# reglab/aquaculture

Measured on AMD Instinct MI355X. Metric: 640px tiles/sec (whole node) YOLOv5m bf16, higher is better.
Workload: dtype bf16

## Files before the change

### aquaculture_amd/csrc/conv1x1_direct.hip

```cpp
#include "conv_device.h"

using namespace aqdev;

namespace {

struct C1Params {
    const char* in;
    char* out;
    const char* w;
    const float* bias;
    const char* zero;
    int in_ld_b, out_ld_b;
    int npix, n_tiles, act;
    float out_inv_scale;
};

constexpr int kNW = 12;

template <int KS, int MBT, int MBW, int NBW> struct C1Geom {
    static constexpr int CIN = 32 * KS, COUT = 16 * MBT, CB = CIN / 8;
    static constexpr int MG = MBT / MBW;
    static constexpr int PG = kNW / MG;
    static constexpr int TP = PG * NBW * 16;
    static constexpr int SPP = CB + 2;
    static constexpr int PXB = SPP * 16;
    static constexpr int NQ = (TP * SPP + 63) / 64;
    static constexpr int XPB = NQ * 1024;
    static constexpr int LDS = 2 * XPB + COUT * 4;
    static constexpr int NST = NBW;
    static_assert(MBT % MBW == 0 && kNW % MG == 0 && LDS <= 160 * 1024, "shape");
};

__device__ __forceinline__ f32x4 c1_silu4(f32x4 v) {
    const f32x4 t = v * -1.44269504f;
    f32x4 d = {__builtin_amdgcn_exp2f(t[0]), __builtin_amdgcn_exp2f(t[1]), __builtin_amdgcn_exp2f(t[2]), __builtin_amdgcn_exp2f(t[3])};
    d = d + 1.0f;
    const f32x4 r = {__builtin_amdgcn_rcpf(d[0]), __builtin_amdgcn_rcpf(d[1]), __builtin_amdgcn_rcpf(d[2]), __builtin_amdgcn_rcpf(d[3])};
    return v * r;
}

template <int KS, int MBT, int MBW, int NBW, bool F8OUT = false>
__global__ __launch_bounds__(kNW * 64) void conv1x1_direct_kernel(const C1Params p) {
    using G = C1Geom<KS, MBT, MBW, NBW>;
    extern __shared__ __attribute__((aligned(16))) char smem[];
    float* s_b = (float*)(smem + 2 * G::XPB);

    const int tid = threadIdx.x, lane = tid & 63;
    const int wave = __builtin_amdgcn_readfirstlane(tid >> 6);
    static_assert(MBW == 2, "the paired-row layout below is written for two M blocks per wave");
    const int mb0 = (wave % G::MG) * MBW, pg = wave / G::MG;
    const int g = lane >> 4, l15 = lane & 15;
    const int cbase = mb0 * 16 + g * 8;

    bf16x8 wv[KS][MBW];
#pragma unroll
    for (int s = 0; s < KS; ++s)
#pragma unroll
        for (int m = 0; m < MBW; ++m) wv[s][m] = ((const bf16x8*)p.w)[((size_t)(mb0 + m) * KS + s) * 64 + lane];
    for (int i = tid; i < G::COUT; i += kNW * 64) s_b[i] = p.bias[i];

    auto issue_dma = [&](int tile, char* xb) {
        const long long n0 = (long long)tile * G::TP;
#pragma unroll 1
        for (int q = wave; q < G::NQ; q += kNW) {
            const int slot = q * 64 + lane;
            const int px = slot / G::SPP, part = slot - px * G::SPP;
            const bool valid = px < G::TP && part < G::CB && n0 + px < p.npix;
            const char* src = p.in + (n0 + px) * p.in_ld_b + part * 16;
            glds16(valid ? src : p.zero, xb + q * 1024);
        }
    };

    int tile = first_tile(gridDim.x, blockIdx.x);
    if (tile < p.n_tiles) issue_dma(tile, smem);
    int cur = 0;
    bool prev_full = false;
    for (; tile < p.n_tiles; tile += gridDim.x, cur ^= 1) {
        const long long n0 = (long long)tile * G::TP;
        const char* s_x = smem + cur * G::XPB;
        if (prev_full) wait_vmcnt<G::NST>(); else wait_vmcnt<0>();
        asm volatile("s_waitcnt lgkmcnt(0)" ::: "memory");
        __builtin_amdgcn_s_barrier();
        asm volatile("" ::: "memory");
        prev_full = n0 + G::TP <= p.npix;
        if (tile + (int)gridDim.x < p.n_tiles) issue_dma(tile + (int)gridDim.x, smem + (cur ^ 1) * G::XPB);

        f32x4 bv[MBW];
#pragma unroll
        for (int m = 0; m < MBW; ++m) bv[m] = *(const f32x4*)(s_b + cbase + m * 4);
        static_assert(G::NST == NBW * 1, "one 16-byte (8-byte with F8OUT) store per pixel block: the wait at the top of the tile loop counts these");
        AQ_STORE_LOOP_UNROLL
// ... 11 lines not shown
#pragma unroll
                for (int m = 0; m < MBW; ++m) acc[m] = __builtin_amdgcn_mfma_f32_16x16x32_bf16(wv[s][m], f[s], acc[m], 0, 0, 0);
            f32x4 v0 = acc[0] + bv[0], v1 = acc[1] + bv[1];
            if (p.act) { v0 = c1_silu4(v0); v1 = c1_silu4(v1); }
            if constexpr (F8OUT) {
                f32x4 q0 = v0 * p.out_inv_scale, q1 = v1 * p.out_inv_scale;
#pragma unroll
                for (int e = 0; e < 4; ++e) {
                    q0[e] = __builtin_amdgcn_fmed3f(q0[e], -448.0f, 448.0f);
                    q1[e] = __builtin_amdgcn_fmed3f(q1[e], -448.0f, 448.0f);
                }
                int w0 = __builtin_amdgcn_cvt_pk_fp8_f32(q0[0], q0[1], 0, false);
                w0 = __builtin_amdgcn_cvt_pk_fp8_f32(q0[2], q0[3], w0, true);
                int w1 = __builtin_amdgcn_cvt_pk_fp8_f32(q1[0], q1[1], 0, false);
                w1 = __builtin_amdgcn_cvt_pk_fp8_f32(q1[2], q1[3], w1, true);
                if (n0 + px < p.npix) *(uint2*)(p.out + (n0 + px) * p.out_ld_b + cbase) = make_uint2((unsigned)w0, (unsigned)w1);
            } else if (n0 + px < p.npix)
                *(uint4*)(p.out + (n0 + px) * p.out_ld_b + cbase * 2) =
                    make_uint4(pack_bf16x2(v0[0], v0[1]), pack_bf16x2(v0[2], v0[3]), pack_bf16x2(v1[0], v1[1]), pack_bf16x2(v1[2], v1[3]));
        }
    }
}

template <int KS, int MBT, int MBW, int NBW, bool F8OUT = false>
int launch_c1(C1Params p, hipStream_t stream) {
    using G = C1Geom<KS, MBT, MBW, NBW>;
    auto fn = conv1x1_direct_kernel<KS, MBT, MBW, NBW, F8OUT>;
    int cus = 0;
    AQ_CHECK_HIP(aq_kernel_lds((const void*)fn, G::LDS));
    AQ_CHECK_HIP(aq_cus(&cus));
    p.n_tiles = (p.npix + G::TP - 1) / G::TP;
    long long grid = cus;
    if (grid > p.n_tiles) grid = p.n_tiles;
    hipLaunchKernelGGL(fn, dim3((unsigned)grid), dim3(kNW * 64), G::LDS, stream, p);
    AQ_CHECK_HIP(hipGetLastError());
    return AQ_OK;
}

}

extern "C" int aq_conv1x1_direct_supported(int cin, int cout) {
    return (cin == 96 && cout == 96) || (cin == 192 && cout == 192) || (cin == 384 && (cout == 192 || cout == 384));
}

extern "C" int aq_pack_conv1x1_direct(const float* w_host, int cin, int cout, void* packed_dev, size_t* bytes, void* stream) {
    AQ_REQUIRE(w_host && bytes && aq_conv1x1_direct_supported(cin, cout), "pack_conv1x1_direct: unsupported %d -> %d", cin, cout);
    const int ks = cin / 32, mbt = cout / 16;
    *bytes = (size_t)mbt * ks * 64 * 16;
    if (!packed_dev) return AQ_OK;
    bf16_t* host = (bf16_t*)calloc(1, *bytes);
    AQ_REQUIRE(host, "pack_conv1x1_direct: out of host memory");
    for (int mb = 0; mb < mbt; ++mb)
        for (int s = 0; s < ks; ++s)
            for (int lane = 0; lane < 64; ++lane) {
                const int r = lane & 15, g = lane >> 4;
                const int co = (mb >> 1) * 32 + 8 * (r >> 2) + 4 * (mb & 1) + (r & 3);
                bf16_t* dst = host + (((size_t)mb * ks + s) * 64 + lane) * 8;
                for (int e = 0; e < 8; ++e) dst[e] = aq_f2bf(w_host[(size_t)co * cin + 32 * s + 8 * g + e]);
            }
    hipError_t e = hipMemcpyAsync(packed_dev, host, *bytes, hipMemcpyHostToDevice, (hipStream_t)stream);
    if (e == hipSuccess) e = hipStreamSynchronize((hipStream_t)stream);
    free(host);
    AQ_CHECK_HIP(e);
    return AQ_OK;
}

extern "C" int aq_conv1x1_direct(const void* in_dev, int in_ld, int in_choff, void* out_dev, int out_ld, int out_choff, int cin, int cout,
                                 const void* packed_w_dev, const float* bias_dev, long long npix, int act, void* stream) {
    AQ_REQUIRE(in_dev && out_dev && packed_w_dev && bias_dev, "conv1x1_direct: null pointer");
    AQ_REQUIRE(aq_conv1x1_direct_supported(cin, cout), "conv1x1_direct: unsupported %d -> %d", cin, cout);
    AQ_REQUIRE(npix > 0 && sg::conv1x1_direct_fits(npix), "conv1x1_direct: bad pixel count");
    AQ_REQUIRE(in_ld % 8 == 0 && out_ld % 8 == 0 && in_choff % 8 == 0 && out_choff % 8 == 0 && in_choff + cin <= in_ld && out_choff + cout <= out_ld,
               "conv1x1_direct: channel slices must be 8-aligned and inside their rows");
    C1Params p{};
    p.in = (const char*)in_dev + (size_t)in_choff * 2; p.in_ld_b = in_ld * 2;
    p.out = (char*)out_dev + (size_t)out_choff * 2; p.out_ld_b = out_ld * 2;
    p.w = (const char*)packed_w_dev; p.bias = bias_dev;
    p.npix = (int)npix; p.act = act;
    p.zero = aq_zero_page();
    AQ_REQUIRE(p.zero, "conv1x1_direct: zero page allocation failed");
    const hipStream_t st = (hipStream_t)stream;
    if (cin == 96) return launch_c1<3, 6, 2, 4>(p, st);
    if (cin == 192) return launch_c1<6, 12, 2, 4>(p, st);
    if (cout == 192) return launch_c1<12, 12, 2, 2>(p, st);
    return launch_c1<12, 24, 2, 4>(p, st);
}


extern "C" int aq_conv1x1_direct_f8out(const void* in_dev, int in_ld, int in_choff, void* out_dev, int out_pitch_bytes, int out_byte_off, int cin,
                                       int cout, const void* packed_w_dev, const float* bias_dev, long long npix, int act, float out_scale,
                                       void* stream) {
    AQ_REQUIRE(in_dev && out_dev && packed_w_dev && bias_dev, "conv1x1_direct_f8out: null pointer");
    AQ_REQUIRE((cin == 192 && cout == 192) || (cin == 384 && cout == 384), "conv1x1_direct_f8out: unsupported %d -> %d", cin, cout);
    AQ_REQUIRE(npix > 0 && sg::conv1x1_direct_fits(npix) && out_scale > 0.0f, "conv1x1_direct_f8out: bad pixel count or scale");
    AQ_REQUIRE(in_ld % 8 == 0 && in_choff % 8 == 0 && in_choff + cin <= in_ld && out_pitch_bytes % 8 == 0 && out_byte_off % 8 == 0 &&
                   out_byte_off + cout <= out_pitch_bytes, "conv1x1_direct_f8out: slices must be 8-byte aligned and inside their rows");
    C1Params p{};
    p.in = (const char*)in_dev + (size_t)in_choff * 2; p.in_ld_b = in_ld * 2;
    p.out = (char*)out_dev + out_byte_off; p.out_ld_b = out_pitch_bytes;
    p.w = (const char*)packed_w_dev; p.bias = bias_dev;
    p.npix = (int)npix; p.act = act; p.out_inv_scale = 1.0f / out_scale;
    p.zero = aq_zero_page();
    AQ_REQUIRE(p.zero, "conv1x1_direct_f8out: zero page allocation failed");
    const hipStream_t st = (hipStream_t)stream;
    if (cin == 192) return launch_c1<6, 12, 2, 4, true>(p, st);
    return launch_c1<12, 24, 2, 4, true>(p, st);
}
```

### aquaculture_amd/csrc/engine.cpp

```cpp
#include "aq_common.h"
#include <unistd.h>
#include <string>

#include <cstdarg>
#include <cstdio>
#include <cstdlib>
#include <cstring>
#include <string>
#include <atomic>
#include <dlfcn.h>
#include <vector>

namespace {
thread_local char g_err[512] = "";
}

void aq_set_error(const char* fmt, ...) {
    va_list ap;
    va_start(ap, fmt);
    vsnprintf(g_err, sizeof(g_err), fmt, ap);
    va_end(ap);
}

extern "C" const char* aq_last_error(void) { return g_err; }
// ... 115 lines not shown
            }
        }
    }
    *kgroups = kg; *kgroups_pad = kgp; *G = g; *cout_rows = rows;
}

struct TensorPlace { size_t offset = 0; size_t bytes = 0; int h = 0, w = 0, elem = 0; };

}

struct aq_engine {
    int device = 0;
    aq_model_desc desc{};
    std::vector<aq_tensor_desc> tensors;
    std::vector<aq_op_desc> ops;
    std::vector<PackedW> packed;
    std::vector<int> conv_cfg;
    int nms_agnostic = 0;
    unsigned long long nms_cls_lo = ~0ULL, nms_cls_hi = ~0ULL;
    struct Tuned { int B = 0, H = 0, W = 0; std::vector<int> cfg; };
    std::vector<Tuned> tuned;
    int tuned_cur = -1;
    bool tuning = false;
    void* zero_page = nullptr;
    int lay_B = 0, lay_H = 0, lay_W = 0;
    bool lay_aug = false;
    int run_H = 0, run_W = 0;
    std::vector<TensorPlace> place;
    size_t off_pred = 0, off_cand = 0, off_cand_rows = 0, off_cand_count = 0, off_cand_wide = 0, off_nms = 0, off_taps = 0, total_bytes = 0;
    int N = 0;
    aq_augment_pass aug[3] = {};
    std::vector<int> aug_family[3], aug_cfg[3];
    void* last_ws = nullptr;
    const uint8_t* last_tiles = nullptr;
    float* calib_amax = nullptr;
    std::vector<int> last_family, last_cfg;
    bool prof = false;
    int ring = 0;
    long long prof_calls = 0;
    std::vector<hipEvent_t> ev;
};

namespace {

void set_dims(aq_engine* e, int H, int W) {
    for (size_t t = 0; t < e->tensors.size(); ++t) {
// ... 289 lines not shown
            if (!(form || igemm)) return fail(oi, "conv: %lld output pixels are past the implicit-GEMM guard (pixels < 2^24, K groups < 2^15, tile count < 2^31) and no other form takes it", npix);
            break;
        }
        default:
            break;
        }
    }
    return -1;
}

bool c3tail_active(aq_engine* e, int oi, int last, int B) {
    if (!e->packed[oi].w_tail || oi + 1 >= last || e->calib_amax || e->tuning) return false;
    const int ci = oi + 1;
    const PackedW& pc = e->packed[ci];
    if (pc.direct_cfg != AQ_CONV_CFG_DIRECT1X1 || (pc.f8_consumer >= 0 && f8_pair_active(e, pc.f8_consumer, B))) return false;
    const aq_engine::Tuned* tt = tuned_for(e);
    const int cfg = e->conv_cfg[ci] >= 0 ? e->conv_cfg[ci] : tt ? tt->cfg[ci] : -1;
    if (cfg != AQ_CONV_CFG_DIRECT1X1) return false;
    const aq_op_desc& b = e->ops[oi];
    const aq_op_desc& c = e->ops[ci];
    const TensorPlace& pl = e->place[b.src.tensor];
    return aq_bottleneck_c3tail_supported(B, pl.h, pl.w, e->tensors[b.src.tensor].channels, e->tensors[c.src.tensor].channels,
                                          e->tensors[c.dst.tensor].channels) != 0;
}

struct AugRun {
    int pass;
    const aq_augment_pass* ps;
    int H0, W0;
    const aq_tap* ytab;
    const aq_tap* xtab;
};

int run_plan(aq_engine* e, const uint8_t* tiles, int B, int H, int W, void* ws, size_t ws_bytes,
             float* pred_out, aq_det* dets, int32_t* counts, float conf, float iou, int max_det, hipStream_t stream,
             int first = 0, int last = -1, const AugRun* ar = nullptr) {
    AQ_REQUIRE(e && tiles && ws, "infer: null pointer");
    const int n_ops = (int)e->ops.size();
    if (last < 0) last = n_ops;
    AQ_REQUIRE(0 <= first && first <= last && last <= n_ops, "run_ops: range [%d, %d) is not inside the plan's %d ops", first, last, n_ops);
    int rc = AQ_OK;
    if (!ar) {
        rc = layout(e, B, H, W);
        if (rc) return rc;
        if (ws_bytes < e->total_bytes) {
            aq_set_error("workspace too small: need %zu bytes, got %zu", e->total_bytes, ws_bytes);
// ... 5 lines not shown
    const float aug_scale = ar ? ar->ps->scale : 1.0f, aug_flip_w = ar && ar->ps->flip ? (float)ar->W0 : 0.0f;
    e->last_ws = ws; e->last_tiles = tiles;
    const int prec = e->desc.precision;
    const bool whole = first == 0 && last == n_ops;
    hipEvent_t* ev = nullptr;
    if (whole && !ar && e->prof && e->ring > 0) ev = e->ev.data() + (size_t)(e->prof_calls % e->ring) * (n_ops + 1);
    float* pred = pred_out ? pred_out : (float*)((char*)ws + e->off_pred);
    int32_t* cand = (int32_t*)((char*)ws + e->off_cand);
    int32_t* cand_count = (int32_t*)((char*)ws + e->off_cand_count);
    float* cand_rows = (float*)((char*)ws + e->off_cand_rows);
    const char* use_sd = getenv("AQ_STEMDOWN");
    const bool stemdown = use_sd && *use_sd == '1' && prec == AQ_BF16 && n_ops > 2 && e->ops[0].kind == AQ_OP_STEM && e->ops[1].kind == AQ_OP_DOWNBLOCK &&
                          e->ops[0].dst.channels == 48 && e->ops[1].src.tensor == e->ops[0].dst.tensor && e->ops[1].src.ch_off == e->ops[0].dst.ch_off &&
                          aq_stemdown_supported(H, W) && ((uintptr_t)tiles & 3) == 0 && !scaled;
    const bool fuse_heads = dets != nullptr && heads_fused(e);
    bool heads_started = ar != nullptr;
    int heads_done = 0;
    for (int oi = 0; oi < first; ++oi)
        if (fuse_heads && e->ops[oi].kind == AQ_OP_CONV && e->ops[oi].level >= 0) {
            heads_started = true;
            ++heads_done;
        }
    int tail_conv = -1;
    for (int oi = first; oi < last; ++oi) {
        const aq_op_desc& op = e->ops[oi];
        if (ev) AQ_CHECK_HIP(hipEventRecord(ev[oi], stream));
        const bool mark = g_roctx.on();
        if (mark) {
            char name[96];
            snprintf(name, sizeof name, "aq op %02d kind %d: %d -> %d ch, k%d s%d%s", oi, op.kind, op.src.channels, op.dst.channels, op.k, op.stride,
                     op.level >= 0 ? " (detect head)" : "");
            g_roctx.push(name);
        }
        switch (op.kind) {
        case AQ_OP_PREPROCESS:
            if (scaled)
                rc = aq_preprocess_s2d_scaled(tiles, ar->H0, ar->W0, ar->ytab, ar->xtab, ar->ps->h, ar->ps->w, tptr(e, ws, tiles, op.dst.tensor), B, H, W,
                                              prec, stream);
            else
                rc = aq_preprocess_s2d(tiles, tptr(e, ws, tiles, op.dst.tensor), B, H, W, prec, stream);
            break;
        case AQ_OP_CONV:
            if (oi == tail_conv) {
                note_launch(e, oi, AQ_FAM_DIRECT1X1, AQ_CONV_CFG_DIRECT1X1);
                break;
            }
            if (ar && op.level >= 0 && !((ar->ps->level_mask >> op.level) & 1)) {
                note_launch(e, oi, AQ_FAM_NONE);
                break;
            }
            if (fuse_heads && op.level >= 0) {
                int32_t* wide = (int32_t*)((char*)ws + e->off_cand_wide);
                if (!heads_started) {
                    AQ_CHECK_HIP(hipMemsetAsync(wide, 0, sizeof(int32_t) * B * kCountStride, stream));
                    heads_started = true;
                }
                const TensorPlace& pl = e->place[op.src.tensor];
                int off = 0;
                for (int l = 0; l < op.level; ++l) off += e->desc.na * (H / (int)e->desc.stride[l]) * (W / (int)e->desc.stride[l]);
                float anchors[8 * 2];
                for (int a = 0; a < e->desc.na; ++a) {
                    anchors[2 * a] = e->desc.anchors_px[op.level][a][0];
                    anchors[2 * a + 1] = e->desc.anchors_px[op.level][a][1];
                }
                note_launch(e, oi, AQ_FAM_HEAD_DECODE);
                if (ar) {
                    rc = aq_head_decode_aug(tptr(e, ws, tiles, op.src.tensor), e->tensors[op.src.tensor].channels, op.src.ch_off, op.src.channels,
// ... 45 lines not shown
                               op.src.channels, e->packed[oi].w, e->packed[oi].bias, B, pl.h, pl.w, op.res.tensor >= 0, stream);
            break;
        }
        case AQ_OP_DOWNBLOCK: {
            note_launch(e, oi, AQ_FAM_DOWNBLOCK);
            const TensorPlace& pl = e->place[op.src.tensor];
            if (stemdown && oi == 1) {
                rc = aq_stemdown(tiles, tptr(e, ws, tiles, op.dst.tensor), e->tensors[op.dst.tensor].channels, op.dst.ch_off,
                                 e->packed[0].w, e->packed[0].bias, e->packed[oi].w, e->packed[oi].bias, B, H, W, stream);
                break;
            }
            rc = aq_downblock(tptr(e, ws, tiles, op.src.tensor), e->tensors[op.src.tensor].channels, op.src.ch_off,
                              tptr(e, ws, tiles, op.dst.tensor), e->tensors[op.dst.tensor].channels, op.dst.ch_off,
                              e->packed[oi].w, e->packed[oi].bias, B, pl.h, pl.w, stream);
            break;
        }
        case AQ_OP_SPPF_POOL: {
            const TensorPlace& pl = e->place[op.src.tensor];
            rc = aq_sppf_pool(tptr(e, ws, tiles, op.src.tensor), e->tensors[op.src.tensor].channels, op.src.ch_off,
                              op.src.channels, B, pl.h, pl.w, prec, stream);
            break;
        }
        case AQ_OP_UPSAMPLE2X: {
            const TensorPlace& pl = e->place[op.src.tensor];
            rc = aq_upsample2x(tptr(e, ws, tiles, op.src.tensor), e->tensors[op.src.tensor].channels, op.src.ch_off,
                               tptr(e, ws, tiles, op.dst.tensor), e->tensors[op.dst.tensor].channels, op.dst.ch_off,
                               op.src.channels, B, pl.h, pl.w, prec, stream);
            break;
        }
        case AQ_OP_DECODE: {
            if (fuse_heads) break;
            const float* heads[3];
            for (int l = 0; l < 3; ++l) heads[l] = (const float*)tptr(e, ws, tiles, e->desc.head_tensor[l]);
            float anchors[3 * 8 * 2];
            for (int l = 0; l < 3; ++l)
                for (int a = 0; a < e->desc.na; ++a) {
                    anchors[(l * e->desc.na + a) * 2] = e->desc.anchors_px[l][a][0];
                    anchors[(l * e->desc.na + a) * 2 + 1] = e->desc.anchors_px[l][a][1];
                }
            const bool want_nms = dets != nullptr;
            if (ar) {
                rc = aq_detect_decode_aug(heads, e->tensors[e->desc.head_tensor[0]].channels, B, H, W, e->desc.nc, e->desc.na, anchors,
                                          e->desc.stride, ar->ps->level_mask, aug_base, e->N, aug_scale, aug_flip_w, want_nms ? nullptr : pred,
                                          conf, want_nms ? cand : nullptr, want_nms ? cand_rows : nullptr, want_nms ? cand_count : nullptr,
                                          e->N, stream);
                break;
// ... 164 lines not shown
    case AQ_SG_IGEMM: return sg::igemm_fits(v[0], v[1], v[2], v[3], v[4], v[5]);
    case AQ_SG_HEAD_DECODE: return sg::head_decode_fits(v[0], v[1], v[2]);
    case AQ_SG_TILE_BYTES: return sg::tile_bytes_fit(v[0], v[1], v[2]);
    }
    return -1;
}

extern "C" int aq_engine_create(const aq_model_desc* d, int device, aq_engine** out) {
    AQ_REQUIRE(d && out, "engine_create: null pointer");
    AQ_REQUIRE(d->n_ops > 0 && d->n_tensors > 0 && d->ops && d->tensors, "engine_create: empty plan");
    AQ_REQUIRE(d->nl == 3 && d->na >= 1 && d->na <= 8 && d->nc >= 1, "engine_create: unsupported head nl=%d na=%d nc=%d", d->nl, d->na, d->nc);
    AQ_REQUIRE(d->nc <= 128, "engine_create: nc = %d, the NMS class filter covers at most 128 classes", d->nc);
    AQ_REQUIRE(d->precision == AQ_BF16 || d->precision == AQ_FP32 || d->precision == AQ_BF16_W8 || d->precision == AQ_F16X3,
               "engine_create: bad precision %d", d->precision);
    {
        static std::atomic<int> first_device{-1};
        int expected = -1;
        if (!first_device.compare_exchange_strong(expected, device))
            AQ_REQUIRE(expected == device, "engine_create: this process already runs engines on device %d; device %d needs its own process", expected, device);
    }
    AQ_CHECK_HIP(hipSetDevice(device));
    aq_engine* e = new aq_engine();
    e->device = device;
    aq_model_desc compute_desc = *d;
    const bool w8 = d->precision == AQ_BF16_W8;
    if (w8) compute_desc.precision = AQ_BF16;
    const bool x3 = d->precision == AQ_F16X3;
    if (x3) compute_desc.precision = AQ_FP32;
    d = &compute_desc;
    e->desc = *d;
    e->tensors.assign(d->tensors, d->tensors + d->n_tensors);
    e->ops.assign(d->ops, d->ops + d->n_ops);
    e->desc.tensors = e->tensors.data();
    e->desc.ops = e->ops.data();
    e->packed.resize(e->ops.size());
    e->conv_cfg.assign(e->ops.size(), -1);
    const int eb = aq_elem_bytes(d->precision);
    auto fail = [&](int rc) { aq_engine_destroy(e); return rc; };
    if (hipMalloc(&e->zero_page, 4096) != hipSuccess || hipMemset(e->zero_page, 0, 4096) != hipSuccess) {
        aq_set_error("engine_create: zero page allocation failed");
        return fail(AQ_ERR_NOMEM);
    }
    const char* use_tail = getenv("AQ_C3TAIL");
    for (size_t oi = 0; d->precision == AQ_BF16 && !(use_tail && *use_tail == '0') && oi + 1 < e->ops.size(); ++oi) {
        const aq_op_desc& b = e->ops[oi];
        const aq_op_desc& c = e->ops[oi + 1];
// ... 562 lines not shown
```

### aquaculture_amd/engine.py

```python
from __future__ import annotations

import ctypes as C
import os
import re
from typing import Dict, List, Optional, Sequence, Tuple

import numpy as np
import torch

from . import spec as _spec
from .checkpoint import Checkpoint, pack_plan_weights

AQ_BF16, AQ_FP32, AQ_BF16_W8, AQ_F16X3 = 0, 1, 2, 3
PRECISIONS = {"bf16": AQ_BF16, "fp32": AQ_FP32, "fp8w": AQ_BF16, "f16x3": AQ_F16X3}
"""Compute precision of the single-op helpers.  fp8w = fp8 (OCP e4m3fn) weights with per-output-channel power-of-two scales, bf16
activations (quant.py): values bf16 holds exactly, so every bf16 kernel runs them as they are."""
ENGINE_PRECISIONS = {"bf16": AQ_BF16, "fp32": AQ_FP32, "fp8w": AQ_BF16_W8, "f16x3": AQ_F16X3, "fp8": AQ_BF16}
"""aq_model_desc.precision.  AQ_BF16_W8 computes as AQ_BF16; kernels with an fp8-weight stream (the planar 3x3) load the e4m3 codes."""
_DTYPE_CODE = {"act": 0, "f32": 1, "u8": 2}

LIB_PATH = os.path.join(os.path.dirname(os.path.abspath(__file__)), "csrc", "libaqengine.so")


class aq_tensor_desc(C.Structure):
# ... 9 lines not shown
                ("k", C.c_int32), ("stride", C.c_int32), ("pad", C.c_int32), ("act", C.c_int32),
                ("level", C.c_int32), ("weight", C.POINTER(C.c_float)), ("bias", C.POINTER(C.c_float)),
                ("flops_per_tile", C.c_double)]


class aq_model_desc(C.Structure):
    _fields_ = [("precision", C.c_int32), ("nc", C.c_int32), ("na", C.c_int32), ("nl", C.c_int32),
                ("anchors_px", C.c_float * 2 * 8 * 3), ("stride", C.c_float * 3),
                ("head_tensor", C.c_int32 * 3), ("input_tensor", C.c_int32),
                ("n_tensors", C.c_int32), ("n_ops", C.c_int32),
                ("tensors", C.POINTER(aq_tensor_desc)), ("ops", C.POINTER(aq_op_desc))]


class aq_det(C.Structure):
    _fields_ = [("x1", C.c_float), ("y1", C.c_float), ("x2", C.c_float), ("y2", C.c_float),
                ("conf", C.c_float), ("cls", C.c_float)]


EXPORTS = (
    "aq_last_error", "aq_version", "aq_engine_create", "aq_engine_destroy", "aq_engine_workspace_bytes", "aq_size_guard",
    "aq_engine_infer", "aq_engine_run_ops", "aq_engine_candidates", "aq_engine_forward_raw", "aq_engine_tensor_ptr", "aq_engine_profile",
    "aq_engine_op_times", "aq_engine_num_ops", "aq_engine_set_conv_config", "aq_engine_autotune", "aq_engine_set_tuned_table",
    "aq_engine_get_conv_config", "aq_conv_num_configs", "aq_debug_conv_stamp", "aq_debug_mfma_peak",
    "aq_conv_config_tiles", "aq_pack_conv_weights", "aq_pack_conv_weights_x3", "aq_conv2d", "aq_pack_stem_weights", "aq_stem_conv", "aq_pack_bottleneck_weights", "aq_bottleneck", "aq_bottleneck_asm_form", "aq_bottleneck_c3tail_supported", "aq_pack_bottleneck_c3tail_weights", "aq_bottleneck_c3tail", "aq_pack_downblock_weights", "aq_downblock", "aq_stemdown_supported", "aq_stemdown", "aq_conv1x1_direct_supported", "aq_pack_conv1x1_direct", "aq_conv1x1_direct", "aq_conv1x1_asm_supported", "aq_pack_conv1x1_asm", "aq_conv1x1_asm", "aq_nms_opts", "aq_engine_set_nms_options",
    "aq_conv3x3s2_direct_supported", "aq_pack_conv3x3s2_direct", "aq_conv3x3s2_direct",
    "aq_conv3x3_pl_supported", "aq_conv3x3_pl_asm_family", "aq_pack_conv3x3_pl", "aq_conv3x3_pl", "aq_conv3x3_pl_s2_supported", "aq_pack_conv3x3_pl_s2", "aq_conv3x3_pl_s2", "aq_jpeg_scratch_bytes", "aq_jpeg_idct_rgb", "aq_jpeg_idct_rgb_checked", "aq_f32_to_e4m3", "aq_conv1x1_direct_f8out", "aq_absmax_bf16", "aq_engine_calibrate_amax", "aq_engine_set_fp8_scales", "aq_engine_last_launch", "aq_conv3x3_pl_f8_supported", "aq_pack_conv3x3_pl_f8", "aq_conv3x3_pl_f8", "aq_conv3x3_pl_w8_supported", "aq_pack_conv3x3_pl_w8", "aq_conv3x3_pl_w8", "aq_head_decode_supported", "aq_pack_head_weights", "aq_head_decode", "aq_head_counts_gather", "aq_preprocess_s2d", "aq_sppf_pool",
    "aq_upsample2x", "aq_letterbox_u8", "aq_letterbox_tiles_u8", "aq_format_label_rows", "aq_detect_decode", "aq_nms_scratch_bytes", "aq_nms", "aq_jpeg_huffman_decode", "aq_write_label_files",
    "aq_crop_jpeg_coefs", "aq_crop_jpeg_bytes", "aq_write_crop_files",
    "aq_annotate_u8", "aq_image_jpeg_coefs", "aq_image_jpeg_bytes", "aq_write_image_files",
    "aq_blank_stats_scratch_bytes", "aq_blank_stats_u8",
    "aq_blank_geom_scratch_bytes", "aq_blank_components_u8", "aq_blank_ring_edges_u8",
    "aq_facility_scratch_bytes", "aq_facility_dbscan_f64",
    "aq_land_scratch_bytes", "aq_land_filter_f64",
    "aq_land_images_scratch_bytes", "aq_land_images_f64",
    "aq_eval_scratch_bytes", "aq_eval_member_conf_f64", "aq_box_match_f64",
    "aq_eval_subsets_scratch_bytes", "aq_eval_member_conf_subsets_f64", "aq_box_match_subsets_scratch_bytes", "aq_box_match_subsets_f64",
    "aq_model_error_match_f64", "aq_model_error_moments_f64",
    "aq_tonnage_simulate_f64", "aq_tonnage_reduce_f64", "aq_tonnage_ndtri_f64", "aq_tonnage_uniform_f64",
    "aq_bernoulli_counts_i32",
    "aq_depth_ranges_f64", "aq_depth_stats_f64",
    "aq_dedup_fill_u32", "aq_dedup_sets_u32", "aq_dedup_select_f64",
    "aq_coverage_first_i32",
    "aq_overlap_partners_f64", "aq_overlap_clip_f64",
    "aq_facility_bounds_f64", "aq_box_join_count_i32", "aq_box_join_list_i32",
    "aq_augment_geometry", "aq_augment_taps", "aq_stem_conv_scaled", "aq_preprocess_s2d_scaled", "aq_head_decode_aug", "aq_detect_decode_aug",
    "aq_engine_workspace_bytes_augment", "aq_engine_infer_augment", "aq_engine_forward_raw_augment", "aq_engine_last_launch_augment",
)
# ... 85 lines not shown
    lib.aq_engine_set_fp8_scales.argtypes = [vp, C.POINTER(f32), i32]
    lib.aq_conv1x1_direct_f8out.argtypes = [vp, i32, i32, vp, i32, i32, i32, i32, vp, vp, C.c_longlong, i32, f32, vp]
    lib.aq_absmax_bf16.argtypes = [vp, i32, i32, i32, C.c_longlong, vp, vp]
    lib.aq_debug_conv_stamp.argtypes = [vp, sz]
    lib.aq_debug_mfma_peak.argtypes = [i32, i32, vp, vp]
    lib.aq_conv_config_tiles.argtypes = [i32, C.POINTER(i32), C.POINTER(i32)]
    lib.aq_pack_conv_weights.argtypes = [C.POINTER(f32), i32, i32, i32, i32, vp, C.POINTER(sz), vp]
    lib.aq_pack_conv_weights_x3.argtypes = [C.POINTER(f32), C.POINTER(f32), i32, i32, i32, vp, C.POINTER(sz), vp, C.POINTER(sz), vp]
    lib.aq_conv2d.argtypes = [vp, i32, i32, i32, vp, i32, i32, i32, vp, i32, i32, vp, vp,
                              i32, i32, i32, i32, i32, i32, i32, i32, i32, vp, vp]
    lib.aq_pack_stem_weights.argtypes = [C.POINTER(f32), i32, i32, vp, C.POINTER(sz), vp]
    lib.aq_stem_conv.argtypes = [vp, vp, i32, i32, i32, vp, vp, i32, i32, i32, i32, i32, vp]
    lib.aq_pack_bottleneck_weights.argtypes = [C.POINTER(f32), C.POINTER(f32), i32, vp, C.POINTER(sz), vp]
    lib.aq_bottleneck.argtypes = [vp, i32, i32, vp, i32, i32, i32, vp, vp, i32, i32, i32, i32, vp]
    lib.aq_bottleneck_asm_form.argtypes = [i32] * 6
    lib.aq_bottleneck_c3tail_supported.argtypes = [i32, i32, i32, i32, i32, i32]
    lib.aq_pack_bottleneck_c3tail_weights.argtypes = [C.POINTER(f32), C.POINTER(f32), C.POINTER(f32), vp, C.POINTER(sz), vp]
    lib.aq_bottleneck_c3tail.argtypes = [vp, i32, i32, vp, i32, i32, vp, i32, i32, vp, vp, i32, i32, i32, i32, vp]
    lib.aq_pack_downblock_weights.argtypes = [C.POINTER(f32), C.POINTER(f32), vp, C.POINTER(sz), vp]
    lib.aq_downblock.argtypes = [vp, i32, i32, vp, i32, i32, vp, vp, i32, i32, i32, vp]
    lib.aq_conv1x1_direct_supported.argtypes = [i32, i32]
    lib.aq_pack_conv1x1_direct.argtypes = [C.POINTER(f32), i32, i32, vp, C.POINTER(sz), vp]
    lib.aq_conv1x1_direct.argtypes = [vp, i32, i32, vp, i32, i32, i32, i32, vp, vp, C.c_longlong, i32, vp]
    lib.aq_nms_opts.argtypes = [vp, i32, i32, i32, i32, f32, f32, i32, vp, vp, i32, vp, vp, vp, i32, C.c_ulonglong, C.c_ulonglong, vp]
    lib.aq_engine_set_nms_options.argtypes = [vp, i32, C.c_ulonglong, C.c_ulonglong]
    lib.aq_conv1x1_asm_supported.argtypes = [i32, i32]
    lib.aq_pack_conv1x1_asm.argtypes = [C.POINTER(f32), i32, i32, vp, C.POINTER(sz), vp]
    lib.aq_conv1x1_asm.argtypes = [vp, i32, i32, vp, i32, i32, i32, i32, vp, vp, C.c_longlong, i32, vp]
    lib.aq_conv3x3s2_direct_supported.argtypes = [i32, i32]
    lib.aq_pack_conv3x3s2_direct.argtypes = [C.POINTER(f32), i32, i32, vp, C.POINTER(sz), vp]
    lib.aq_conv3x3s2_direct.argtypes = [vp, i32, i32, vp, i32, i32, i32, i32, vp, vp, i32, i32, i32, i32, vp]
    lib.aq_conv3x3_pl_supported.argtypes = [i32, i32]
    lib.aq_conv3x3_pl_asm_family.argtypes = [i32]
    lib.aq_pack_conv3x3_pl.argtypes = [C.POINTER(f32), i32, i32, vp, C.POINTER(sz), vp]
    lib.aq_conv3x3_pl.argtypes = [vp, C.c_longlong, C.c_longlong, i32, vp, i32, i32, i32, vp, i32, i32, vp, vp, i32, i32, i32, i32, vp]
    lib.aq_conv3x3_pl_w8.argtypes = lib.aq_conv3x3_pl.argtypes
    lib.aq_pack_conv3x3_pl_w8.argtypes = [C.POINTER(C.c_float), C.POINTER(C.c_float), i32, i32, vp, C.POINTER(C.c_size_t), vp, vp]
    lib.aq_conv3x3_pl_w8_supported.argtypes = [i32] * 5
    lib.aq_jpeg_scratch_bytes.argtypes = [i32, i32, i32]
    lib.aq_jpeg_scratch_bytes.restype = sz
    lib.aq_jpeg_idct_rgb.argtypes = [vp, vp, vp, i32, i32, i32, vp, vp, vp]
    lib.aq_jpeg_idct_rgb_checked.argtypes = [vp, vp, vp, i32, i32, i32, vp, vp, vp, vp]
    lib.aq_f32_to_e4m3.argtypes = [f32]
    lib.aq_f32_to_e4m3.restype = C.c_ubyte
    lib.aq_conv3x3_pl_f8_supported.argtypes = [i32] * 5
    lib.aq_pack_conv3x3_pl_f8.argtypes = [C.POINTER(f32), C.POINTER(f32), i32, i32, f32, vp, C.POINTER(sz), vp, vp]
# ... 2161 lines not shown
```

### include/aq_engine.h

```cpp
#ifndef AQ_ENGINE_H
#define AQ_ENGINE_H

#include <stddef.h>
#include <stdint.h>

#ifdef __cplusplus
extern "C" {
#endif

typedef enum aq_status {
    AQ_OK = 0,
    AQ_ERR_INVALID = -1,
    AQ_ERR_HIP = -2,
    AQ_ERR_NOMEM = -3,
    AQ_ERR_WORKSPACE = -4
} aq_status;

typedef enum aq_precision {
    AQ_BF16 = 0,
    AQ_FP32 = 1,
    AQ_BF16_W8 = 2,
    AQ_F16X3 = 3
} aq_precision;

// ... 130 lines not shown
                  const void* packed_w_dev, const float* bias_dev, int B, int H, int W, int shortcut, void* stream);
int aq_bottleneck_asm_form(int C, int B, int H, int W, int in_ld, int out_ld);

int aq_bottleneck_c3tail_supported(int B, int H, int W, int in_ld, int cat_ld, int out_ld);
int aq_pack_bottleneck_c3tail_weights(const float* w1_host, const float* w2_host, const float* w3_host, void* packed_dev, size_t* bytes,
                                      void* stream);
int aq_bottleneck_c3tail(const void* in_dev, int in_ld, int in_choff, const void* cat_dev, int cat_ld, int cat_choff, void* out_dev,
                         int out_ld, int out_choff, const void* packed_w_dev, const float* bias_dev, int B, int H, int W, int shortcut,
                         void* stream);

int aq_pack_downblock_weights(const float* wa_host, const float* wb_host, void* packed_dev, size_t* bytes, void* stream);
int aq_downblock(const void* in_dev, int in_ld, int in_choff, void* out_dev, int out_ld, int out_choff,
                 const void* packed_w_dev, const float* bias_dev, int B, int H, int W, void* stream);
int aq_stemdown_supported(int Hi, int Wi);
int aq_stemdown(const uint8_t* tiles_dev, void* out_dev, int out_ld, int out_choff, const void* stem_w_dev, const float* stem_bias_dev,
                const void* packed_w_dev, const float* bias_dev, int B, int Hi, int Wi, void* stream);

#define AQ_CONV_CFG_DIRECT1X1 1000
#define AQ_CONV_CFG_ONE_TILE_PER_WG 4096
int aq_conv1x1_direct_supported(int cin, int cout);
int aq_pack_conv1x1_direct(const float* w_host, int cin, int cout, void* packed_dev, size_t* bytes, void* stream);
int aq_conv1x1_direct(const void* in_dev, int in_ld, int in_choff, void* out_dev, int out_ld, int out_choff, int cin, int cout,
                      const void* packed_w_dev, const float* bias_dev, long long npix, int act, void* stream);

#define AQ_CONV_CFG_ASM1X1 1004
int aq_conv1x1_asm_supported(int cin, int cout);
int aq_pack_conv1x1_asm(const float* w_host, int cin, int cout, void* packed_dev, size_t* bytes, void* stream);
int aq_conv1x1_asm(const void* in_dev, int in_ld, int in_choff, void* out_dev, int out_ld, int out_choff, int cin, int cout,
                   const void* packed_w_dev, const float* bias_dev, long long npix, int act, void* stream);

#define AQ_CONV_CFG_DIRECT3X3S2 1001
int aq_conv3x3s2_direct_supported(int cin, int cout);
int aq_pack_conv3x3s2_direct(const float* w_host, int cin, int cout, void* packed_dev, size_t* bytes, void* stream);
int aq_conv3x3s2_direct(const void* in_dev, int in_ld, int in_choff, void* out_dev, int out_ld, int out_choff, int cin, int cout,
                        const void* packed_w_dev, const float* bias_dev, int B, int H, int W, int act, void* stream);
#define AQ_CONV_CFG_PL3X3 1002
int aq_conv3x3_pl_supported(int cin, int cout);
int aq_conv3x3_pl_asm_family(int nb);
int aq_pack_conv3x3_pl(const float* w_krsc_host, int cin, int cout, void* packed_dev, size_t* bytes, void* stream);
int aq_conv3x3_pl(const void* in_dev, long long in_pixel_stride_b, long long in_group_stride_b, int cin,
                  void* out_dev, int out_ld, int out_choff, int cout, const void* res_dev, int res_ld, int res_choff,
                  const void* packed_w_dev, const float* bias_dev, int B, int H, int W, int act, void* stream);
#define AQ_CONV_CFG_PL3X3S2 1003
int aq_conv3x3_pl_s2_supported(int cin, int cout, int B, int H, int W);
int aq_pack_conv3x3_pl_s2(const float* w_krsc_host, int cin, int cout, void* packed_dev, size_t* bytes, void* stream);
int aq_conv3x3_pl_s2(const void* in_dev, int in_ld, int in_choff, int cin, void* out_dev, int out_ld, int out_choff, int cout,
// ... 228 lines not shown
```

Before: 16820.

## Fold nearest 2x upsample into following 1x1 conv DMA and add 6-wave variant

When an UPSAMPLE2X op feeds only the low half of a concat consumed by a 384->192 1x1 conv, the upsample launch is skipped. The conv's load stage instead reads those channels directly from the low-resolution tensor, using magic-number division to map each output pixel to its source. This removes one kernel launch and a full write/read of the upsampled tensor. It also adds an optional 6-wave kernel form with an occupancy-based grid, which is off by default and selected through an env var, plus a query API.

```diff
diff --git a/aquaculture_amd/csrc/conv1x1_direct.hip b/aquaculture_amd/csrc/conv1x1_direct.hip
--- a/aquaculture_amd/csrc/conv1x1_direct.hip
+++ b/aquaculture_amd/csrc/conv1x1_direct.hip
@@ -13,14 +13,19 @@
     int in_ld_b, out_ld_b;
     int npix, n_tiles, act;
     float out_inv_scale;
+    const char* lo;
+    int lo_ld_b;
+    int w2;
+    unsigned w2_mul;
+    int w2_shift;
 };
 
 constexpr int kNW = 12;
 
-template <int KS, int MBT, int MBW, int NBW> struct C1Geom {
+template <int KS, int MBT, int MBW, int NBW, int NW = kNW> struct C1Geom {
     static constexpr int CIN = 32 * KS, COUT = 16 * MBT, CB = CIN / 8;
     static constexpr int MG = MBT / MBW;
-    static constexpr int PG = kNW / MG;
+    static constexpr int PG = NW / MG;
     static constexpr int TP = PG * NBW * 16;
     static constexpr int SPP = CB + 2;
     static constexpr int PXB = SPP * 16;
@@ -28,7 +33,7 @@
     static constexpr int XPB = NQ * 1024;
     static constexpr int LDS = 2 * XPB + COUT * 4;
     static constexpr int NST = NBW;
-    static_assert(MBT % MBW == 0 && kNW % MG == 0 && LDS <= 160 * 1024, "shape");
+    static_assert(MBT % MBW == 0 && NW % MG == 0 && LDS <= 160 * 1024, "shape");
 };
 
 __device__ __forceinline__ f32x4 c1_silu4(f32x4 v) {
@@ -39,9 +44,9 @@
     return v * r;
 }
 
-template <int KS, int MBT, int MBW, int NBW, bool F8OUT = false>
-__global__ __launch_bounds__(kNW * 64) void conv1x1_direct_kernel(const C1Params p) {
-    using G = C1Geom<KS, MBT, MBW, NBW>;
+template <int KS, int MBT, int MBW, int NBW, bool F8OUT = false, int NW = kNW, bool UP = false>
+__global__ __launch_bounds__(NW * 64, 3) void conv1x1_direct_kernel(const C1Params p) {
+    using G = C1Geom<KS, MBT, MBW, NBW, NW>;
     extern __shared__ __attribute__((aligned(16))) char smem[];
     float* s_b = (float*)(smem + 2 * G::XPB);
 
@@ -57,16 +62,23 @@
     for (int s = 0; s < KS; ++s)
 #pragma unroll
         for (int m = 0; m < MBW; ++m) wv[s][m] = ((const bf16x8*)p.w)[((size_t)(mb0 + m) * KS + s) * 64 + lane];
-    for (int i = tid; i < G::COUT; i += kNW * 64) s_b[i] = p.bias[i];
+    for (int i = tid; i < G::COUT; i += NW * 64) s_b[i] = p.bias[i];
 
     auto issue_dma = [&](int tile, char* xb) {
         const long long n0 = (long long)tile * G::TP;
 #pragma unroll 1
-        for (int q = wave; q < G::NQ; q += kNW) {
+        for (int q = wave; q < G::NQ; q += NW) {
             const int slot = q * 64 + lane;
             const int px = slot / G::SPP, part = slot - px * G::SPP;
             const bool valid = px < G::TP && part < G::CB && n0 + px < p.npix;
             const char* src = p.in + (n0 + px) * p.in_ld_b + part * 16;
+            if constexpr (UP) {
+                if (part < G::CB / 2) {
+                    const unsigned n = (unsigned)(n0 + px);
+                    const unsigned r = (unsigned)(((unsigned long long)n * p.w2_mul) >> p.w2_shift), x = n - r * (unsigned)p.w2;
+                    src = p.lo + ((long long)(r >> 1) * (p.w2 >> 1) + (x >> 1)) * p.lo_ld_b + part * 16;
+                }
+            }
             glds16(valid ? src : p.zero, xb + q * 1024);
         }
     };
@@ -124,19 +136,45 @@
     }
 }
 
-template <int KS, int MBT, int MBW, int NBW, bool F8OUT = false>
+template <int KS, int MBT, int MBW, int NBW, bool F8OUT, int NW, bool UP = false>
+int c1_grid(long long* grid) {
+    using G = C1Geom<KS, MBT, MBW, NBW, NW>;
+    auto fn = conv1x1_direct_kernel<KS, MBT, MBW, NBW, F8OUT, NW, UP>;
+    int cus = 0, occ = 1;
+    AQ_CHECK_HIP(aq_cus(&cus));
+    if constexpr (NW == kNW) AQ_CHECK_HIP(aq_kernel_lds((const void*)fn, G::LDS));
+    else AQ_CHECK_HIP(aq_kernel_blocks((const void*)fn, NW * 64, G::LDS, G::LDS, &occ));
+    *grid = (long long)cus * occ;
+    return AQ_OK;
+}
+
+template <int KS, int MBT, int MBW, int NBW, bool F8OUT = false, int NW = kNW, bool UP = false>
 int launch_c1(C1Params p, hipStream_t stream) {
-    using G = C1Geom<KS, MBT, MBW, NBW>;
-    auto fn = conv1x1_direct_kernel<KS, MBT, MBW, NBW, F8OUT>;
-    int cus = 0;
-    AQ_CHECK_HIP(aq_kernel_lds((const void*)fn, G::LDS));
-    AQ_CHECK_HIP(aq_cus(&cus));
+    using G = C1Geom<KS, MBT, MBW, NBW, NW>;
+    auto fn = conv1x1_direct_kernel<KS, MBT, MBW, NBW, F8OUT, NW, UP>;
+    long long grid = 0;
+    if (const int rc = c1_grid<KS, MBT, MBW, NBW, F8OUT, NW, UP>(&grid)) return rc;
     p.n_tiles = (p.npix + G::TP - 1) / G::TP;
-    long long grid = cus;
     if (grid > p.n_tiles) grid = p.n_tiles;
-    hipLaunchKernelGGL(fn, dim3((unsigned)grid), dim3(kNW * 64), G::LDS, stream, p);
+    hipLaunchKernelGGL(fn, dim3((unsigned)grid), dim3(NW * 64), G::LDS, stream, p);
     AQ_CHECK_HIP(hipGetLastError());
     return AQ_OK;
+}
+
+enum C1Shape { kC1_96, kC1_192, kC1_384_192, kC1_192_F8, kC1Shapes };
+constexpr bool kC1SixByDefault[kC1Shapes] = {false, false, false, false};
+
+bool c1_six_waves(C1Shape shape) {
+    const char* e = getenv("AQ_C1_WAVES");
+    const int forced = e ? atoi(e) : 0;
+    return forced == 6 || (forced != 12 && kC1SixByDefault[shape]);
+}
+
+void c1_div_magic(unsigned d, unsigned* mul, int* shift) {
+    int l = 0;
+    while ((1ull << l) < d) ++l;
+    *mul = (unsigned)((1ull << (31 + l)) / d + 1);
+    *shift = 31 + l;
 }
 
 }
@@ -182,10 +220,28 @@
     p.zero = aq_zero_page();
     AQ_REQUIRE(p.zero, "conv1x1_direct: zero page allocation failed");
     const hipStream_t st = (hipStream_t)stream;
+    if (cin == 96 && c1_six_waves(kC1_96)) return launch_c1<3, 6, 2, 4, false, 6>(p, st);
+    if (cin == 192 && c1_six_waves(kC1_192)) return launch_c1<6, 12, 2, 4, false, 6>(p, st);
+    if (cin == 384 && cout == 192 && c1_six_waves(kC1_384_192)) return launch_c1<12, 12, 2, 2, false, 6>(p, st);
     if (cin == 96) return launch_c1<3, 6, 2, 4>(p, st);
     if (cin == 192) return launch_c1<6, 12, 2, 4>(p, st);
     if (cout == 192) return launch_c1<12, 12, 2, 2>(p, st);
     return launch_c1<12, 24, 2, 4>(p, st);
+}
+
+extern "C" int aq_conv1x1_direct_form(int cin, int cout, int f8out, int* waves, int* tile_pixels, long long* max_grid) {
+    AQ_REQUIRE(waves && tile_pixels && max_grid, "conv1x1_direct_form: null pointer");
+    AQ_REQUIRE(f8out ? (cin == 192 && cout == 192) || (cin == 384 && cout == 384) : aq_conv1x1_direct_supported(cin, cout),
+               "conv1x1_direct_form: unsupported %d -> %d", cin, cout);
+#define C1_FORM(KS, MBT, MBW, NBW, F8, NW) \
+    (*waves = NW, *tile_pixels = C1Geom<KS, MBT, MBW, NBW, NW>::TP, c1_grid<KS, MBT, MBW, NBW, F8, NW>(max_grid))
+    if (f8out && cin == 192) return c1_six_waves(kC1_192_F8) ? C1_FORM(6, 12, 2, 4, true, 6) : C1_FORM(6, 12, 2, 4, true, kNW);
+    if (f8out) return C1_FORM(12, 24, 2, 4, true, kNW);
+    if (cin == 96) return c1_six_waves(kC1_96) ? C1_FORM(3, 6, 2, 4, false, 6) : C1_FORM(3, 6, 2, 4, false, kNW);
+    if (cin == 192) return c1_six_waves(kC1_192) ? C1_FORM(6, 12, 2, 4, false, 6) : C1_FORM(6, 12, 2, 4, false, kNW);
+    if (cout == 192) return c1_six_waves(kC1_384_192) ? C1_FORM(12, 12, 2, 2, false, 6) : C1_FORM(12, 12, 2, 2, false, kNW);
+    return C1_FORM(12, 24, 2, 4, false, kNW);
+#undef C1_FORM
 }
 
 
@@ -205,6 +261,35 @@
     p.zero = aq_zero_page();
     AQ_REQUIRE(p.zero, "conv1x1_direct_f8out: zero page allocation failed");
     const hipStream_t st = (hipStream_t)stream;
+    if (cin == 192 && c1_six_waves(kC1_192_F8)) return launch_c1<6, 12, 2, 4, true, 6>(p, st);
     if (cin == 192) return launch_c1<6, 12, 2, 4, true>(p, st);
     return launch_c1<12, 24, 2, 4, true>(p, st);
 }
+
+
+extern "C" int aq_conv1x1_direct_up2x_supported(int cin, int cout) { return cin == 384 && cout == 192; }
+
+extern "C" int aq_conv1x1_direct_up2x(const void* lo_dev, int lo_ld, int lo_choff, const void* cat_dev, int cat_ld, int cat_choff, void* out_dev,
+                                      int out_ld, int out_choff, int cin, int cout, const void* packed_w_dev, const float* bias_dev, int B, int H,
+                                      int W, int act, void* stream) {
+    AQ_REQUIRE(lo_dev && cat_dev && out_dev && packed_w_dev && bias_dev, "conv1x1_direct_up2x: null pointer");
+    AQ_REQUIRE(aq_conv1x1_direct_up2x_supported(cin, cout), "conv1x1_direct_up2x: unsupported %d -> %d", cin, cout);
+    const long long npix = 4LL * B * H * W;
+    AQ_REQUIRE(B > 0 && H > 0 && W > 0 && W < (1 << 24) && sg::conv1x1_direct_fits(npix), "conv1x1_direct_up2x: bad geometry %d x %d x %d", B, H, W);
+    AQ_REQUIRE(lo_ld % 8 == 0 && cat_ld % 8 == 0 && out_ld % 8 == 0 && lo_choff % 8 == 0 && cat_choff % 8 == 0 && out_choff % 8 == 0 &&
+                   lo_choff + cin / 2 <= lo_ld && cat_choff + cin <= cat_ld && out_choff + cout <= out_ld,
+               "conv1x1_direct_up2x: channel slices must be 8-aligned and inside their rows");
+    C1Params p{};
+    p.in = (const char*)cat_dev + (size_t)cat_choff * 2; p.in_ld_b = cat_ld * 2;
+    p.lo = (const char*)lo_dev + (size_t)lo_choff * 2; p.lo_ld_b = lo_ld * 2;
+    p.w2 = 2 * W;
+    c1_div_magic((unsigned)p.w2, &p.w2_mul, &p.w2_shift);
+    p.out = (char*)out_dev + (size_t)out_choff * 2; p.out_ld_b = out_ld * 2;
+    p.w = (const char*)packed_w_dev; p.bias = bias_dev;
+    p.npix = (int)npix; p.act = act;
+    p.zero = aq_zero_page();
+    AQ_REQUIRE(p.zero, "conv1x1_direct_up2x: zero page allocation failed");
+    const hipStream_t st = (hipStream_t)stream;
+    if (c1_six_waves(kC1_384_192)) return launch_c1<12, 12, 2, 2, false, 6, true>(p, st);
+    return launch_c1<12, 12, 2, 2, false, kNW, true>(p, st);
+}
diff --git a/aquaculture_amd/csrc/engine.cpp b/aquaculture_amd/csrc/engine.cpp
--- a/aquaculture_amd/csrc/engine.cpp
+++ b/aquaculture_amd/csrc/engine.cpp
@@ -161,6 +161,7 @@
     std::vector<Tuned> tuned;
     int tuned_cur = -1;
     bool tuning = false;
+    bool upfold = true;
     void* zero_page = nullptr;
     int lay_B = 0, lay_H = 0, lay_W = 0;
     bool lay_aug = false;
@@ -496,6 +497,32 @@
     const TensorPlace& pl = e->place[b.src.tensor];
     return aq_bottleneck_c3tail_supported(B, pl.h, pl.w, e->tensors[b.src.tensor].channels, e->tensors[c.src.tensor].channels,
                                           e->tensors[c.dst.tensor].channels) != 0;
+}
+
+bool upfold_active(aq_engine* e, int oi, int last, int B) {
+    if (!e->upfold || e->desc.precision != AQ_BF16 || oi + 1 >= last || e->calib_amax || e->tuning) return false;
+    const int ci = oi + 1;
+    const aq_op_desc& u = e->ops[oi];
+    const aq_op_desc& c = e->ops[ci];
+    if (c.kind != AQ_OP_CONV || c.k != 1 || c.stride != 1 || c.level >= 0 || c.res.tensor >= 0) return false;
+    if (u.src.channels != u.dst.channels || c.src.tensor != u.dst.tensor || c.src.ch_off != u.dst.ch_off || c.src.channels != 2 * u.dst.channels) return false;
+    const PackedW& pc = e->packed[ci];
+    if (pc.direct_cfg != AQ_CONV_CFG_DIRECT1X1 || !pc.w_direct || (pc.f8_consumer >= 0 && f8_pair_active(e, pc.f8_consumer, B))) return false;
+    const aq_engine::Tuned* tt = tuned_for(e);
+    const int cfg = e->conv_cfg[ci] >= 0 ? e->conv_cfg[ci] : tt ? tt->cfg[ci] : -1;
+    if (cfg != AQ_CONV_CFG_DIRECT1X1 || !aq_conv1x1_direct_up2x_supported(c.src.channels, c.dst.channels)) return false;
+    const TensorPlace& pd = e->place[c.dst.tensor];
+    if (!sg::conv1x1_direct_fits((long long)B * pd.h * pd.w)) return false;
+    const TensorPlace& pl = e->place[u.src.tensor];
+    if (pd.h != 2 * pl.h || pd.w != 2 * pl.w) return false;
+    auto reads_up = [&](const aq_slice& s) {
+        return s.tensor == u.dst.tensor && s.ch_off < u.dst.ch_off + u.dst.channels && s.ch_off + s.channels > u.dst.ch_off;
+    };
+    for (int oj = ci + 1; oj < (int)e->ops.size(); ++oj)
+        if (reads_up(e->ops[oj].src) || reads_up(e->ops[oj].res)) return false;
+    for (int l = 0; l < e->desc.nl; ++l)
+        if (e->desc.head_tensor[l] == u.dst.tensor) return false;
+    return true;
 }
 
 struct AugRun {
@@ -547,6 +574,7 @@
             ++heads_done;
         }
     int tail_conv = -1;
+    int up_conv = -1;
     for (int oi = first; oi < last; ++oi) {
         const aq_op_desc& op = e->ops[oi];
         if (ev) AQ_CHECK_HIP(hipEventRecord(ev[oi], stream));
@@ -568,6 +596,16 @@
         case AQ_OP_CONV:
             if (oi == tail_conv) {
                 note_launch(e, oi, AQ_FAM_DIRECT1X1, AQ_CONV_CFG_DIRECT1X1);
+                break;
+            }
+            if (oi == up_conv) {
+                const aq_op_desc& u = e->ops[oi - 1];
+                const TensorPlace& pl = e->place[u.src.tensor];
+                note_launch(e, oi, AQ_FAM_DIRECT1X1, AQ_CONV_CFG_DIRECT1X1);
+                rc = aq_conv1x1_direct_up2x(tptr(e, ws, tiles, u.src.tensor), e->tensors[u.src.tensor].channels, u.src.ch_off,
+                                            tptr(e, ws, tiles, op.src.tensor), e->tensors[op.src.tensor].channels, op.src.ch_off,
+                                            tptr(e, ws, tiles, op.dst.tensor), e->tensors[op.dst.tensor].channels, op.dst.ch_off,
+                                            op.src.channels, op.dst.channels, e->packed[oi].w_direct, e->packed[oi].bias, B, pl.h, pl.w, op.act, stream);
                 break;
             }
             if (ar && op.level >= 0 && !((ar->ps->level_mask >> op.level) & 1)) {
@@ -659,6 +697,10 @@
             break;
         }
         case AQ_OP_UPSAMPLE2X: {
+            if (upfold_active(e, oi, last, B)) {
+                up_conv = oi + 1;
+                break;
+            }
             const TensorPlace& pl = e->place[op.src.tensor];
             rc = aq_upsample2x(tptr(e, ws, tiles, op.src.tensor), e->tensors[op.src.tensor].channels, op.src.ch_off,
                                tptr(e, ws, tiles, op.dst.tensor), e->tensors[op.dst.tensor].channels, op.dst.ch_off,
@@ -869,6 +911,10 @@
     AQ_CHECK_HIP(hipSetDevice(device));
     aq_engine* e = new aq_engine();
     e->device = device;
+    {
+        const char* uf = getenv("AQ_UPFOLD");
+        e->upfold = !(uf && *uf == '0');
+    }
     aq_model_desc compute_desc = *d;
     const bool w8 = d->precision == AQ_BF16_W8;
     if (w8) compute_desc.precision = AQ_BF16;
diff --git a/aquaculture_amd/engine.py b/aquaculture_amd/engine.py
--- a/aquaculture_amd/engine.py
+++ b/aquaculture_amd/engine.py
@@ -55,7 +55,7 @@
     "aq_engine_infer", "aq_engine_run_ops", "aq_engine_candidates", "aq_engine_forward_raw", "aq_engine_tensor_ptr", "aq_engine_profile",
     "aq_engine_op_times", "aq_engine_num_ops", "aq_engine_set_conv_config", "aq_engine_autotune", "aq_engine_set_tuned_table",
     "aq_engine_get_conv_config", "aq_conv_num_configs", "aq_debug_conv_stamp", "aq_debug_mfma_peak",
-    "aq_conv_config_tiles", "aq_pack_conv_weights", "aq_pack_conv_weights_x3", "aq_conv2d", "aq_pack_stem_weights", "aq_stem_conv", "aq_pack_bottleneck_weights", "aq_bottleneck", "aq_bottleneck_asm_form", "aq_bottleneck_c3tail_supported", "aq_pack_bottleneck_c3tail_weights", "aq_bottleneck_c3tail", "aq_pack_downblock_weights", "aq_downblock", "aq_stemdown_supported", "aq_stemdown", "aq_conv1x1_direct_supported", "aq_pack_conv1x1_direct", "aq_conv1x1_direct", "aq_conv1x1_asm_supported", "aq_pack_conv1x1_asm", "aq_conv1x1_asm", "aq_nms_opts", "aq_engine_set_nms_options",
+    "aq_conv_config_tiles", "aq_pack_conv_weights", "aq_pack_conv_weights_x3", "aq_conv2d", "aq_pack_stem_weights", "aq_stem_conv", "aq_pack_bottleneck_weights", "aq_bottleneck", "aq_bottleneck_asm_form", "aq_bottleneck_c3tail_supported", "aq_pack_bottleneck_c3tail_weights", "aq_bottleneck_c3tail", "aq_pack_downblock_weights", "aq_downblock", "aq_stemdown_supported", "aq_stemdown", "aq_conv1x1_direct_supported", "aq_pack_conv1x1_direct", "aq_conv1x1_direct", "aq_conv1x1_direct_form", "aq_conv1x1_direct_up2x_supported", "aq_conv1x1_direct_up2x", "aq_conv1x1_asm_supported", "aq_pack_conv1x1_asm", "aq_conv1x1_asm", "aq_nms_opts", "aq_engine_set_nms_options",
     "aq_conv3x3s2_direct_supported", "aq_pack_conv3x3s2_direct", "aq_conv3x3s2_direct",
     "aq_conv3x3_pl_supported", "aq_conv3x3_pl_asm_family", "aq_pack_conv3x3_pl", "aq_conv3x3_pl", "aq_conv3x3_pl_s2_supported", "aq_pack_conv3x3_pl_s2", "aq_conv3x3_pl_s2", "aq_jpeg_scratch_bytes", "aq_jpeg_idct_rgb", "aq_jpeg_idct_rgb_checked", "aq_f32_to_e4m3", "aq_conv1x1_direct_f8out", "aq_absmax_bf16", "aq_engine_calibrate_amax", "aq_engine_set_fp8_scales", "aq_engine_last_launch", "aq_conv3x3_pl_f8_supported", "aq_pack_conv3x3_pl_f8", "aq_conv3x3_pl_f8", "aq_conv3x3_pl_w8_supported", "aq_pack_conv3x3_pl_w8", "aq_conv3x3_pl_w8", "aq_head_decode_supported", "aq_pack_head_weights", "aq_head_decode", "aq_head_counts_gather", "aq_preprocess_s2d", "aq_sppf_pool",
     "aq_upsample2x", "aq_letterbox_u8", "aq_letterbox_tiles_u8", "aq_format_label_rows", "aq_detect_decode", "aq_nms_scratch_bytes", "aq_nms", "aq_jpeg_huffman_decode", "aq_write_label_files",
@@ -187,6 +187,9 @@
     lib.aq_conv1x1_direct_supported.argtypes = [i32, i32]
     lib.aq_pack_conv1x1_direct.argtypes = [C.POINTER(f32), i32, i32, vp, C.POINTER(sz), vp]
     lib.aq_conv1x1_direct.argtypes = [vp, i32, i32, vp, i32, i32, i32, i32, vp, vp, C.c_longlong, i32, vp]
+    lib.aq_conv1x1_direct_form.argtypes = [i32, i32, i32, C.POINTER(i32), C.POINTER(i32), C.POINTER(C.c_longlong)]
+    lib.aq_conv1x1_direct_up2x_supported.argtypes = [i32, i32]
+    lib.aq_conv1x1_direct_up2x.argtypes = [vp, i32, i32, vp, i32, i32, vp, i32, i32, i32, i32, vp, vp, i32, i32, i32, i32, vp]
     lib.aq_nms_opts.argtypes = [vp, i32, i32, i32, i32, f32, f32, i32, vp, vp, i32, vp, vp, vp, i32, C.c_ulonglong, C.c_ulonglong, vp]
     lib.aq_engine_set_nms_options.argtypes = [vp, i32, C.c_ulonglong, C.c_ulonglong]
     lib.aq_conv1x1_asm_supported.argtypes = [i32, i32]
diff --git a/include/aq_engine.h b/include/aq_engine.h
--- a/include/aq_engine.h
+++ b/include/aq_engine.h
@@ -176,6 +176,11 @@
 int aq_pack_conv1x1_direct(const float* w_host, int cin, int cout, void* packed_dev, size_t* bytes, void* stream);
 int aq_conv1x1_direct(const void* in_dev, int in_ld, int in_choff, void* out_dev, int out_ld, int out_choff, int cin, int cout,
                       const void* packed_w_dev, const float* bias_dev, long long npix, int act, void* stream);
+int aq_conv1x1_direct_form(int cin, int cout, int f8out, int* waves, int* tile_pixels, long long* max_grid);
+int aq_conv1x1_direct_up2x_supported(int cin, int cout);
+int aq_conv1x1_direct_up2x(const void* lo_dev, int lo_ld, int lo_choff, const void* cat_dev, int cat_ld, int cat_choff, void* out_dev,
+                           int out_ld, int out_choff, int cin, int cout, const void* packed_w_dev, const float* bias_dev, int B, int H,
+                           int W, int act, void* stream);
 
 #define AQ_CONV_CFG_ASM1X1 1004
 int aq_conv1x1_asm_supported(int cin, int cout);
```

Result: faster. 17000 (median of 6 runs) (+1.0%).
